# Nico59000/Ternary-image-codec

Measured on AMD Instinct MI355X. Metric: Mpix/s encode+decode 8K RS(26,20), higher is better.
Workload: dtype u8

## Files before the change

### ternary-image-codec_amd/csrc/t3_api_decode.cpp

```cpp
#include <hip/hip_runtime.h>
#include <math.h>
#include <stdio.h>
#include <string.h>

#include <stdlib.h>

#include <algorithm>
#include <mutex>
#include <vector>

#include "../../include/t3hip.h"
#include "t3_ctx.hpp"
#include "t3_decode.h"
#include "t3_host.hpp"
#include "t3_repair.h"
#include "t3_window.h"

using namespace t3;

namespace {
struct HdrCheck { HdrExpect ex; uint32_t hs; uint32_t* verdict; const uint8_t* in; };

int launch_hdr_compare(const HdrCheck* h, hipStream_t s) {
    if (!h) return T3_OK;
// ... 19 lines not shown
        HIPCHK(hipMemcpy(tab.synd_lut[ki], img.data(), tab.synd_lut_bytes[ki], hipMemcpyHostToDevice));
    }
    if (!tab.roots[ki]) {
        const Field& F = field(); const int t = (26 - k) / 2;
        size_t n = 1; for (int i = 0; i < t; ++i) n *= 27;
        std::vector<uint32_t> tbl(n);
        for (size_t idx = 0; idx < n; ++idx) {
            uint8_t sg[5] = {1, 0, 0, 0, 0}; { size_t v = idx; for (int q = 1; q <= t; ++q) { sg[q] = (uint8_t)(v % 27); v /= 27; } }
            uint32_t mask = 0;
            for (int i = 0; i < 26; ++i) {
                const uint8_t x = F.t.exp[i == 0 ? 0 : 26 - i];
                uint8_t acc = sg[t];
                for (int q = t - 1; q >= 0; --q) acc = F.t.add[F.t.mul[acc * 27 + x] * 27 + sg[q]];
                if (acc == 0) mask |= 1u << i;
            }
            tbl[idx] = mask;
        }
        HIPCHK(hipMalloc((void**)&tab.roots[ki], n * 4));
        HIPCHK(hipMemcpy(tab.roots[ki], tbl.data(), n * 4, hipMemcpyHostToDevice));
    }
    if (!tab.synd_afrag[ki]) {
        std::vector<uint32_t> af; build_mfma_syndrome(k, af);
        HIPCHK(hipMalloc((void**)&tab.synd_afrag[ki], af.size() * 4)); HIPCHK(hipMemcpy(tab.synd_afrag[ki], af.data(), af.size() * 4, hipMemcpyHostToDevice));
    }
    if (!tab.synd_T) {
        std::vector<uint32_t> img; build_syndrome_T(img);
        HIPCHK(hipMalloc((void**)&tab.synd_T, img.size() * 4)); HIPCHK(hipMemcpy(tab.synd_T, img.data(), img.size() * 4, hipMemcpyHostToDevice));
        build_syndrome_T(img, 16);
        HIPCHK(hipMalloc((void**)&tab.synd_T16, img.size() * 4)); HIPCHK(hipMemcpy(tab.synd_T16, img.data(), img.size() * 4, hipMemcpyHostToDevice));
        uint8_t sm[kFx2SmallBytes + kFx2ModBytes]; build_fx2_small(sm); build_fx2_mod(sm + kFx2SmallBytes);
        HIPCHK(hipMalloc((void**)&tab.fx2_small, sizeof sm)); HIPCHK(hipMemcpy(tab.fx2_small, sm, sizeof sm, hipMemcpyHostToDevice));
    }
    if (!tab.fma) {
        const Field& F = field();
        std::vector<uint8_t> t(19696, 0);
        for (int x = 0; x < 27; ++x) for (int y = 0; y < 27; ++y) for (int c = 0; c < 27; ++c) t[(size_t)(x * 27 + y) * 27 + c] = F.t.add[c * 27 + F.t.mul[x * 27 + y]];
        HIPCHK(hipMalloc((void**)&tab.fma, t.size())); HIPCHK(hipMemcpy(tab.fma, t.data(), t.size(), hipMemcpyHostToDevice));
    }
    return T3_OK;
}

int rgb_dequant_tables(Ctx& c, const uint8_t** out) {
    uint8_t*& d = c.rgb.dequant;
    if (!d) {
        uint8_t t[328]; memset(t, 0, sizeof t);
        auto cl = [](long v) { return v < 0 ? 0 : (v > 255 ? 255 : v); };
        for (int q = 0; q <= 242; ++q) t[q] = (uint8_t)cl(lround(q * (255.0 / 242.0)));
        for (int q = -40; q <= 40; ++q) t[244 + q + 40] = (uint8_t)cl(lround(128 + q * (128.0 / 40.0)));
        HIPCHK(hipMalloc((void**)&d, sizeof t)); HIPCHK(hipMemcpy(d, t, sizeof t, hipMemcpyHostToDevice));
    }
    *out = d; return T3_OK;
}

template <class A> void scrambler_rows(A& a, const ScrCycle& sc) {
    uint8_t rows[12][16]; memset(rows, 0, sizeof rows);
    for (int r = 0; r < 11; ++r) for (int q = 0; q < 13; ++q) rows[r][q] = (uint8_t)(27u * sc.cyc[(r + q) % 6]);
    for (int q = 0; q < 13; ++q) rows[11][q] = (uint8_t)(27u * (q == 0 ? sc.pre[0] : q == 1 ? sc.pre[1] : sc.cyc[(4 + q) % 6]));
    static_assert(sizeof a.pat == sizeof rows, "pattern rows");
    memcpy(a.pat, rows, sizeof rows);
}


struct FusedPlan { DecFx2Args a; const void* fn; uint32_t grid, threads; bool tickets, whole_frame; };
int plan_fixed_fused(uint64_t body_bytes, uint32_t hdr_syms, const t3_layout& L, const ScrCycle& sc, void* d_out, uint64_t units, int to_pixels,
                     uint32_t* d_fail, FusedPlan& p, uint32_t bcn_slot = 0, uint32_t bcn_period = 0, uint32_t tile_lo = 0, uint32_t tile_hi = 0xFFFFFFFFu) {
    if (L.interleave2d || L.n_raw_words == 0) return 1;
    Ctx& c = ctx(); const DecodeTables& tab = c.dec;
    std::lock_guard<std::mutex> lk(c.tab_mu);
    if (!single_k(L)) return 1;
// ... 820 lines not shown
```

### ternary-image-codec_amd/csrc/t3_decode_fx2.h

```cpp
#pragma once
#include "t3_decode_fx.h"
#include "t3_host.hpp"

namespace t3 {
namespace {

__device__ __forceinline__ uint32_t mod26(uint32_t u) { return min(u, u + 26u); }

struct Synd { uint32_t lo, hi; };

typedef uint32_t Geo;
struct Blk { bool valid, first; uint32_t c0, off, yb; };
constexpr uint32_t kFx2Dummy = 384;

template <int R>
__device__ __forceinline__ Geo fx2_geo(const uint32_t item, const uint32_t n_items, const uint32_t nb, const DevDiv& div_nb, const uint32_t tile0, uint32_t& off0) {
    constexpr uint32_t K = 26 - R;
    const uint32_t bi = min(div_ge2(item, div_nb), 8u), m = item - bi * nb;
    const uint32_t m3 = m - 3u * ((m * 683u) >> 11);
    const Row rw = row(bi);
    uint32_t cb = rw.boff6 + 2u * m3; cb -= cb >= 6u ? 6u : 0u;
    off0 = (uint32_t)rw.body_off + 26u * (tile0 * nb + m);
    return (bi + 9u * K * m) | cb << 16 | (item < n_items ? 1u << 19 : 0u);
}
template <int R>
__device__ __forceinline__ bool fx2_has_block(const Geo g, const uint32_t tile, const uint32_t n_tiles, const uint32_t nb) {
    constexpr uint32_t K = 26 - R;
    bool v = (g >> 19) != 0u;
    if (tile + 1u >= n_tiles) {
        const uint32_t yr = g & 0xFFFFu, m = yr / (9u * K), bi = yr - 9u * K * m;
        v = v && tile * nb + m < row(bi).blocks;
    }
    return v;
}
__device__ __forceinline__ Blk fx2_block(const Geo g, const uint32_t off, const bool valid, const uint32_t u2, const uint32_t y_off) {
// ... 75 lines not shown
    const auto sw = __builtin_amdgcn_permlane32_swap(Pown, Pown, false, false);
    Synd r; r.lo = sw[0]; r.hi = sw[1];
    if constexpr (RM != R) {
        const uint64_t V = (uint64_t)sw[0] | (uint64_t)sw[1] << (8u * H);
        constexpr uint64_t M = (1ull << (8u * HB)) - 1ull;
        r.lo = (uint32_t)(V & M); r.hi = (uint32_t)((V >> (8u * HB)) & M);
    }
    return r;
}

template <int R, uint32_t SMB = 0>
__device__ __forceinline__ uint32_t fx2_single(const Synd& sy, const uint32_t yb, const uint32_t FMA) {
    constexpr uint32_t SM = SMB + kFx2Small;
    constexpr uint32_t K = 26 - R, H = R / 2;
    uint32_t lg[R]; bool ok = true;
#pragma unroll
    for (uint32_t j = 0; j < (uint32_t)R; ++j) {
        const uint32_t s = ((j < H ? sy.lo : sy.hi) >> (8u * (j % H))) & 0xFFu;
        lg[j] = lds_u8(SM + kFx2LG + s);
        ok = ok && lg[j] != 0xFFu;
    }
    const uint32_t p = mod26(lg[1] - lg[0]);
#pragma unroll
    for (uint32_t j = 1; j + 1 < (uint32_t)R; ++j) ok = ok && mod26(lg[j + 1] - lg[j]) == p;
    if (!ok) return 0u;
    if (p < K) {
        const uint32_t m = lds_u8(SM + kFx2EX + mod26(lg[0] - p));
        const uint32_t ad = yb + 9u * p;
        *T3_LDS(uint8_t, ad) = (uint8_t)lds_u8(FMA + (2u * 27u + m) * 27u + lds_u8(ad));
    }
    return 1u;
}

template <int R, uint32_t SMB = 0, bool WIDE = true>
__device__ __forceinline__ uint32_t fx2_correct(const uint32_t* S, Fix& fx, const uint32_t* __restrict__ root_tbl, const uint32_t FMA) {
    constexpr uint32_t SM = SMB + kFx2Small;
    constexpr int T = R / 2;
    auto tab = [](uint32_t idx) -> uint32_t { return lds_u8(idx); };
    uint32_t Sx[R];
#pragma unroll
    for (int j = 0; j < R; ++j) Sx[j] = __umul24(S[j], 729u) + FMA;
    uint32_t sg[T + 1], sg27[T + 1], bs27[T + 1];
#pragma unroll
    for (int i = 0; i <= T; ++i) { sg[i] = 0; sg27[i] = 0; bs27[i] = 0; }
    sg[0] = 1; sg27[0] = 27; bs27[1] = 27u * 2u;
    uint32_t L = 0;
    bool over = false;
#pragma unroll
    for (int n = 0; n < R; ++n) {
        uint32_t d = S[n];
#pragma unroll
        for (int i = 1; i <= T; ++i) if (i <= n) d = tab(Sx[n - i] + sg27[i] + d);
        const bool upd = d != 0 && 2u * L <= (uint32_t)n;
        const uint32_t dx = __umul24(d, 729u) + FMA;
        uint32_t old27[T + 1];
#pragma unroll
        for (int i = 0; i <= T; ++i) old27[i] = sg27[i];
#pragma unroll
        for (int i = 1; i <= T; ++i) if (i <= n + 1) { sg[i] = tab(dx + bs27[i] + sg[i]); sg27[i] = 27u * sg[i]; }
        const uint32_t ninv = lds_u8(SM + kFx2NINV + d), nix = __umul24(ninv, 729u) + FMA;
        uint32_t nb27[T + 1];
        nb27[0] = 0; nb27[1] = 27u * ninv;
#pragma unroll
        for (int i = 2; i <= T; ++i) nb27[i] = (i <= n + 1) ? 27u * tab(nix + old27[i - 1]) : 0u;
        if (upd) { L = (uint32_t)n + 1u - L; over = over || L > (uint32_t)T; }
#pragma unroll
        for (int i = T; i >= 1; --i) bs27[i] = upd ? nb27[i] : bs27[i - 1];
        bs27[0] = 0;
    }
    uint32_t deg = 0;
#pragma unroll
    for (int i = 1; i <= T; ++i) if (sg[i] != 0) deg = (uint32_t)i;
    if (over || deg != L) return 1u;
    uint32_t ridx = sg[T];
#pragma unroll
    for (int q = T - 1; q >= 1; --q) ridx = ridx * 27u + sg[q];
    const uint32_t roots = root_tbl[ridx];
    const uint32_t np = (uint32_t)__popc(roots);
    if (np != deg) return 1u;
    uint32_t Om[T];
#pragma unroll
    for (int q = 0; q < T; ++q) {
        uint32_t acc = S[q];
#pragma unroll
        for (int j = 1; j <= q; ++j) acc = tab(Sx[q - j] + sg27[j] + acc);
        Om[q] = acc;
    }
    uint32_t s22 = 0;
    if constexpr (T >= 2) s22 = tab(FMA + 729u + sg27[2] + sg[2]);
    const uint32_t s22_27 = 27u * s22;
    if constexpr (WIDE) {
        uint32_t r = roots, bad = 0u;
        uint32_t pe[T], xix[T];
    #pragma unroll
        for (int e = 0; e < T; ++e) {
            const bool have = (uint32_t)e < np;
            const uint32_t p = have ? (uint32_t)__ffs((int)r) - 1u : 0u; r &= r - 1u;
            pe[e] = p;
            xix[e] = __umul24(lds_u8(SM + kFx2EX + (p == 0 ? 0u : 26u - p)), 729u) + FMA;
        }
        uint32_t num[T], den[T];
    #pragma unroll
        for (int e = 0; e < T; ++e) { num[e] = Om[T - 1]; den[e] = tab(xix[e] + s22_27 + sg[1]); }
    #pragma unroll
        for (int q = T - 2; q >= 0; --q) {
    #pragma unroll
// ... 2 lines not shown
        if constexpr (T >= 4) {
    #pragma unroll
            for (int e = 0; e < T; ++e) { const uint32_t x2 = tab(xix[e] + sg27[4]); const uint32_t x3 = tab(xix[e] + 27u * x2); den[e] = tab(xix[e] + 27u * x3 + den[e]); }
        }
    #pragma unroll
        for (int e = 0; e < T; ++e) {
            const bool have = (uint32_t)e < np;
            bad |= (have && den[e] == 0u) ? 1u : 0u;
            fx.pos[e] = pe[e]; fx.mag[e] = tab(FMA + 729u * lds_u8(SM + kFx2NEG + num[e]) + 27u * lds_u8(SM + kFx2INV + den[e]));
        }
        if (bad) return 1u;
    } else {
        uint32_t r = roots;
#pragma unroll
        for (int e = 0; e < T; ++e) {
            if ((uint32_t)e < np) {
                const uint32_t p = (uint32_t)__ffs((int)r) - 1u; r &= r - 1u;
                const uint32_t xi = lds_u8(SM + kFx2EX + (p == 0 ? 0u : 26u - p));
                const uint32_t xix = __umul24(xi, 729u) + FMA;
                uint32_t num = Om[T - 1];
#pragma unroll
                for (int q = T - 2; q >= 0; --q) num = tab(xix + 27u * num + Om[q]);
                uint32_t den = tab(xix + s22_27 + sg[1]);
                if constexpr (T >= 4) { const uint32_t x2 = tab(xix + sg27[4]); const uint32_t x3 = tab(xix + 27u * x2); den = tab(xix + 27u * x3 + den); }
                if (den == 0) return 1u;
                fx.pos[e] = p; fx.mag[e] = tab(FMA + 729u * lds_u8(SM + kFx2NEG + num) + 27u * lds_u8(SM + kFx2INV + den));
            }
        }
    }
    fx.np = np;
    return 0u;
}

template <int R, uint32_t SMB = 0, bool WIDE = true>
__device__ __forceinline__ bool fx2_fix_block(const uint32_t lo, const uint32_t hi, const uint32_t yb, const uint32_t* __restrict__ root_tbl, const uint32_t FMA) {
    constexpr uint32_t K = 26 - R, H = R / 2;
    uint32_t S[R];
#pragma unroll
    for (uint32_t j = 0; j < (uint32_t)R; ++j) S[j] = ((j < H ? lo : hi) >> (8u * (j % H))) & 0xFFu;
    Fix fx; fx.np = 0;
    if (fx2_correct<R, SMB, WIDE>(S, fx, root_tbl, FMA) != 0u) return false;
    if constexpr (WIDE) {
        uint32_t ad[R / 2], yv[R / 2];
    #pragma unroll
        for (int q = 0; q < R / 2; ++q) { ad[q] = ((uint32_t)q < fx.np && fx.pos[q] < K) ? yb + 9u * fx.pos[q] : SMB + kFx2Dummy + 4u * (uint32_t)q; yv[q] = lds_u8(ad[q]); }
    #pragma unroll
        for (int q = 0; q < R / 2; ++q) yv[q] = lds_u8(FMA + (54u + fx.mag[q]) * 27u + min(yv[q], 26u));
    #pragma unroll
        for (int q = 0; q < R / 2; ++q) *T3_LDS(uint8_t, ad[q]) = (uint8_t)yv[q];
    } else {
#pragma unroll
        for (int q = 0; q < R / 2; ++q)
            if ((uint32_t)q < fx.np && fx.pos[q] < K) { const uint32_t ad = yb + 9u * fx.pos[q]; *T3_LDS(uint8_t, ad) = (uint8_t)lds_u8(FMA + (54u + fx.mag[q]) * 27u + lds_u8(ad)); }
    }
    return true;
}

template <int R, uint32_t SMB = 0, bool WIDE = true>
__device__ __forceinline__ void fx2_own_blocks(const uint32_t* __restrict__ roots, const uint32_t fma_off, uint32_t* fail, const Synd& sA, const Synd& sB, const Blk& bA, const Blk& bB, const uint32_t tag,
                                               const uint32_t lane, const uint32_t cnt_addr, const uint32_t q_off, const uint32_t qcap) {
    const uint32_t h = lane >> 5;
    Synd own; own.lo = h ? sB.lo : sA.lo; own.hi = h ? sB.hi : sA.hi;
    const bool valid = h ? bB.valid : bA.valid;
    const uint32_t yb = h ? bB.yb : bA.yb;
    bool flagged = valid && (own.lo | own.hi) != 0u;
    if (flagged) flagged = fx2_single<R, SMB>(own, yb, fma_off) == 0u;
    const uint64_t bal = __builtin_amdgcn_ballot_w64(flagged);
    if (bal != 0ull) {
        const uint32_t cnt = (uint32_t)__popcll(bal), first = (uint32_t)__builtin_ctzll(bal);
        uint32_t base = 0;
        if (__builtin_amdgcn_mbcnt_hi(~0u, __builtin_amdgcn_mbcnt_lo(~0u, 0u)) == first) base = __hip_atomic_fetch_add((uint32_t*)__builtin_assume_aligned(lds + cnt_addr, 4), cnt, __ATOMIC_RELAXED, __HIP_MEMORY_SCOPE_WORKGROUP);
        base = __builtin_amdgcn_readlane(base, (int)first);
        if (flagged) {
            const uint32_t slot = base + __builtin_amdgcn_mbcnt_hi((uint32_t)(bal >> 32), __builtin_amdgcn_mbcnt_lo((uint32_t)bal, 0u));
            if (__builtin_expect(slot < qcap, 1)) {
                *T3_LDS(u32x2, q_off + 8u * slot) = u32x2{own.lo, own.hi};
                *T3_LDS(uint16_t, q_off + 8u * qcap + 2u * slot) = (uint16_t)tag;
            } else if (!fx2_fix_block<R, SMB, WIDE>(own.lo, own.hi, yb, roots, fma_off)) atomicAdd(fail, 1u);
        }
    }
}

template <int R, uint32_t SMB = 0, bool WIDE = true>
__device__ __forceinline__ void fx2_queue_entry(const uint32_t* __restrict__ roots, const uint32_t fma_off, uint32_t* fail, const uint32_t e, const uint32_t q_off, const uint32_t qcap, const uint32_t y_off) {
    const u32x2 sy = *T3_LDS(const u32x2, q_off + 8u * e);
    const uint32_t tag = *T3_LDS(const uint16_t, q_off + 8u * qcap + 2u * e);
    if (!fx2_fix_block<R, SMB, WIDE>(sy.x, sy.y, y_off + tag, roots, fma_off)) atomicAdd(fail, 1u);
}

}
}
```

### ternary-image-codec_amd/csrc/t3_decode_uep.hip

```cpp
#include <hip/hip_runtime.h>
#include <stdint.h>

#include "../../include/t3hip.h"
#include "t3_decode.h"
#include "t3_decode_fx.h"
#include "t3_decode_fx2.h"
#include "t3_decode_wg.h"

namespace t3 {

namespace {

constexpr uint32_t kUepCnt = 144;
struct GrpRec { uint32_t r, nb, n_items, af_off, q_rel, q_cap, div_mul, div_sh; uint8_t bands[12]; uint32_t pad_; };
static_assert(sizeof(GrpRec) == 48, "group record");

__device__ __forceinline__ IlRow row_at(const DecUepArgs& a, uint32_t v) { return il_row_of<div_ge2>(v, a.n_sym, a.il_w, a.il_A, a.div_A, a.div_w); }
struct Runs { uint32_t at[3], lo[3], len[3], n; };
__device__ __forceinline__ Runs tile_runs(const DecUepArgs& a, const uint32_t S0) {
    Runs R; R.n = 0;
#pragma unroll
    for (int i = 0; i < 3; ++i) { R.at[i] = 0; R.lo[i] = 0; R.len[i] = 0; }
    const uint32_t E = min(S0 + a.TS, a.n_sym);
    if (S0 >= E) return R;
// ... 7 lines not shown
    if (!a.il_on) { push(0u, S0, E - S0); return R; }
    const IlRow r0 = row_at(a, S0), r1 = row_at(a, E - 1u);
    const uint32_t e0 = min(r0.start + r0.len, E);
    push(0u, r0.odd ? 2u * r0.start + r0.len - e0 : S0, e0 - S0);
    if (e0 < E) {
        const uint32_t c0 = max(r1.start, e0);
        push(e0 - S0, e0, c0 - e0);
        push(c0 - S0, r1.odd ? 2u * r1.start + r1.len - E : c0, E - c0);
    }
    return R;
}

__device__ __forceinline__ void px3_from_syms(const uint32_t* s, uint16_t* o) {
    const uint32_t Y0 = s[0] + 27u * (s[1] - 9u * div9(s[1])), B0 = div9(s[1]) + 3u * s[2];
    const uint32_t R0 = s[3] + 27u * (s[4] - 3u * div3(s[4])), Y1 = div3(s[4]) + 9u * s[5];
    const uint32_t B1 = s[6] + 27u * (s[7] - 3u * div3(s[7]));
    const uint32_t R1 = div3(s[7]) + 9u * (s[8] - 9u * div9(s[8]));
    const uint32_t Y2 = div9(s[8]) + 3u * s[9] + 81u * (s[10] - 3u * div3(s[10]));
    const uint32_t B2 = div3(s[10]) + 9u * (s[11] - 9u * div9(s[11])), R2 = div9(s[11]) + 3u * s[12];
    o[0] = (uint16_t)Y0; o[1] = (uint16_t)(B0 - 40u); o[2] = (uint16_t)(R0 - 40u); o[3] = (uint16_t)Y1; o[4] = (uint16_t)(B1 - 40u); o[5] = (uint16_t)(R1 - 40u);
    o[6] = (uint16_t)Y2; o[7] = (uint16_t)(B2 - 40u); o[8] = (uint16_t)(R2 - 40u);
}

template <int R, int RM, bool WIDE>
__device__ __forceinline__ void uep_pass(const DecUepArgs& a, const Geo gA, const Geo gB, const uint32_t offA, const uint32_t offB, const bool vA, const bool vB, const bool haveB,
                                         const uint32_t u2, const uint32_t y_off, const uint32_t (&LA)[4], const uint32_t (&LB)[4], const uint32_t lane,
                                         const uint32_t af_off, const uint32_t* __restrict__ roots, const uint32_t cnt_addr, const uint32_t q_off, const uint32_t q_cap, uint32_t* const failp) {
    constexpr uint32_t TCOP = 16, TBASE = kFx2TPx, MT = kFx2ModPx;
    const uint32_t h = lane >> 5;
    const Blk bA = fx2_block(gA, offA, vA, u2, y_off), bB = fx2_block(gB, offB, vB, u2, y_off);
    const Synd sA = fx2_set<R, TCOP, TBASE, MT, 0, RM>(bA, LA, lane, af_off, a.pat_off);
    Synd sB; sB.lo = 0; sB.hi = 0;
    if (haveB) sB = fx2_set<R, TCOP, TBASE, MT, 0, RM>(bB, LB, lane, af_off, a.pat_off);
    fx2_own_blocks<R, 0, WIDE>(roots, a.fma_off, failp, sA, sB, bA, bB, (h ? gB : gA) & 0xFFFFu, lane, cnt_addr, q_off, q_cap);
}
}

template <int RA, int RB>
__global__ __launch_bounds__(512, 6) void decode_uep_px_kernel(const DecUepArgs a) {
    constexpr uint32_t NW = 4;
    constexpr bool WIDE = !(RA == 6 && RB == 4);
    const uint32_t tid = threadIdx.x, lane = tid & 63u, wave = __builtin_amdgcn_readfirstlane(tid >> 6), nthr = blockDim.x;
    const Tickets tk = tickets_setup(a);
    tk.first(tid);
    uint32_t* const failp = a.verdict ? (uint32_t*)(lds + kFx2FailWg) : a.fail;
    if (tid == 0) *(uint32_t*)(lds + kFx2FailWg) = 0u;
    if (a.verdict && blockIdx.x == 0u && wave == 2u * NW - 1u) {
        uint32_t want = 0;
#pragma unroll
        for (uint32_t q = 0; q < 24; ++q) want = lane == q ? a.hx[q] : want;
        header_check_wave(a, want, lane);
    }
    if (tid == 0) {
        stage_band_rows(a);
#pragma unroll
        for (int i = 0; i < 4; ++i) *(uint32_t*)(lds + kUepCnt + 4 * i) = 0;
        *(uint32_t*)(lds + kFx2Sync) = 0; *(uint32_t*)(lds + kFx2Abort) = 0;
#pragma unroll
        for (int g = 0; g < kUepMaxGrp; ++g) {
            GrpRec r; r.r = a.grp[g].r; r.nb = a.grp[g].nb; r.n_items = a.grp[g].n_items; r.af_off = a.grp[g].af_off; r.q_rel = a.grp[g].q_rel; r.q_cap = a.grp[g].q_cap;
            r.div_mul = a.grp[g].div_nb.mul; r.div_sh = a.grp[g].div_nb.sh; r.pad_ = 0;
#pragma unroll
            for (int q = 0; q < 12; ++q) r.bands[q] = a.grp[g].bands[q];
            *(GrpRec*)(lds + a.rec_off + 48 * g) = r;
        }
#pragma unroll
        for (int i = 0; i < 8; ++i) *(uint32_t*)(lds + a.rec_off + 96 + 4 * i) = a.pair_tab[i];
// ... 62 lines not shown
                    const uint32_t q_rel = __builtin_amdgcn_readfirstlane(*(const uint32_t*)(lds + rb + 16u)), q_cap = __builtin_amdgcn_readfirstlane(*(const uint32_t*)(lds + rb + 20u));
                    const uint32_t toff = tile * 26u * nbg, u2 = 2u * mod3_u32(tile * nbg);
                    uint32_t xa = pass ? xa1 : xa0, xb = pass ? xb1 : xb0, yy = pass ? yy1 : yy0; asm volatile("" : "+v"(xa), "+v"(xb), "+v"(yy));
                    const Geo gA = geo_of(xa, yy, 0), gB = geo_of(xb, yy, 1);
                    const uint32_t oA = (xa & 0x0FFFFFFFu) + toff, oB = (xb & 0x0FFFFFFFu) + toff;
                    const bool vA = has(gA, oA, tile), vB = has(gB, oB, tile), haveB = pip + 32u < n_items;
                    const uint32_t cnt_addr = kUepCnt + 4u * (2u * buf + pgp), q_off = a.q_off + buf * a.q_stride + q_rel;
                    if (pgp == 0u) uep_pass<RA, RA, WIDE>(a, gA, gB, oA, oB, vA, vB, haveB, u2, y_off, LA, LB, lane, af_off, a.grp[0].roots, cnt_addr, q_off, q_cap, failp);
                    else uep_pass<RB, RA, WIDE>(a, gA, gB, oA, oB, vA, vB, haveB, u2, y_off, LA, LB, lane, af_off, a.grp[1].roots, cnt_addr, q_off, q_cap, failp);
                }
            }
            if (tid == 0u) tk.publish(buf, raw, nxt);
            barrier_lds();
            cur = nxt; nxt = tk.next(buf);
        }
        barrier_lds();
    } else {
        const uint32_t cw = wave - NW, ct = cw * 64u + lane;
        uint32_t prev = 0, rdv = 0;
        auto rendezvous = [&]() { consumer_rendezvous<NW>(++rdv, failp, lane); };
        for (uint32_t k = 0;; ++k) {
            if (k >= 1u) {
                const uint32_t tile = prev, buf = (k - 1u) & 1u;
                const uint32_t y_off = a.y_off + buf * a.y_stride, S0 = tile * a.TS;
                {
                    const uint32_t rb1 = a.rec_off + 48u;
                    const uint32_t capA = __builtin_amdgcn_readfirstlane(*(const uint32_t*)(lds + a.rec_off + 20u)), capB = __builtin_amdgcn_readfirstlane(*(const uint32_t*)(lds + rb1 + 20u));
                    const uint32_t qA = a.q_off + buf * a.q_stride + __builtin_amdgcn_readfirstlane(*(const uint32_t*)(lds + a.rec_off + 16u));
                    const uint32_t qB = a.q_off + buf * a.q_stride + __builtin_amdgcn_readfirstlane(*(const uint32_t*)(lds + rb1 + 16u));
                    const uint32_t QA = min(__builtin_amdgcn_readfirstlane(*(const uint32_t*)(lds + kUepCnt + 4u * (2u * buf))), capA);
                    const uint32_t QB = a.n_grp > 1u ? min(__builtin_amdgcn_readfirstlane(*(const uint32_t*)(lds + kUepCnt + 4u * (2u * buf + 1u))), capB) : 0u;
                    const uint32_t nA = (QA + 63u) / 64u, nB = (QB + 63u) / 64u;
                    for (uint32_t sl = cw; sl < nA + nB; sl += NW) {
                        if (sl < nA) { const uint32_t e = 64u * sl + lane; if (e < QA) fx2_queue_entry<RA, 0, WIDE>(a.grp[0].roots, a.fma_off, failp, e, qA, capA, y_off); }
                        else { const uint32_t e = 64u * (sl - nA) + lane; if (e < QB) fx2_queue_entry<RB, 0, WIDE>(a.grp[1].roots, a.fma_off, failp, e, qB, capB, y_off); }
                    }
                }
                rendezvous();
                if (ct < a.n_grp) *(uint32_t*)(lds + kUepCnt + 4u * (2u * buf + ct)) = 0;
                if (a.il_on) {
                    const uint32_t E = min(S0 + a.TS, a.n_sym);
                    for (uint32_t d = ct; 4u * d < a.TS; d += 64u * NW) {
                        const uint32_t v = S0 + 4u * d;
                        if (v >= E) continue;
                        const IlRow rg = row_at(a, v);
                        if (!rg.odd) continue;
                        const uint32_t lo = max(rg.start, S0), hi = min(rg.start + rg.len, E);
                        if ((hi - lo) & 3u) {
                            if (v == lo) for (uint32_t i = lo, j = hi - 1u; i < j; ++i, --j) { const uint32_t x = lds_u8(y_off + (i - S0)); *T3_LDS(uint8_t, y_off + (i - S0)) = (uint8_t)lds_u8(y_off + (j - S0)); *T3_LDS(uint8_t, y_off + (j - S0)) = (uint8_t)x; }
                            continue;
                        }
                        const uint32_t v2 = lo + hi - 4u - v;
                        if (v2 < v) continue;
                        const uint32_t x = *T3_LDS(const uint32_t, y_off + (v - S0)), y = *T3_LDS(const uint32_t, y_off + (v2 - S0));
                        *T3_LDS(uint32_t, y_off + (v - S0)) = __builtin_bswap32(y);
                        if (v2 != v) *T3_LDS(uint32_t, y_off + (v2 - S0)) = __builtin_bswap32(x);
                    }
                    rendezvous();
                }
                const Runs R = tile_runs(a, S0);
                uint32_t j0[3], nu[3], j1[3];
#pragma unroll
                for (int i = 0; i < 3; ++i) { j0[i] = (R.lo[i] + 12u) / 13u; j1[i] = (R.lo[i] + R.len[i]) / 13u; nu[i] = j1[i] > j0[i] ? (j1[i] - j0[i] + 3u) / 4u : 0u; }
                const uint32_t n01 = nu[0] + nu[1], n_all = n01 + nu[2];
                for (uint32_t e = ct; e < n_all; e += 64u * NW) {
                    const uint32_t ri = e < nu[0] ? 0u : e < n01 ? 1u : 2u;
                    const uint32_t eb = ri == 0u ? 0u : ri == 1u ? nu[0] : n01;
                    const uint32_t rj0 = ri == 0u ? j0[0] : ri == 1u ? j0[1] : j0[2], rj1 = ri == 0u ? j1[0] : ri == 1u ? j1[1] : j1[2];
// ... 69 lines not shown
```

### ternary-image-codec_amd/csrc/t3_host.cpp

```cpp
#include "t3_host.hpp"

#include <string.h>

namespace t3 {

namespace {
struct V3 { int t[3]; };
V3 to_v(int s) { return V3{{s % 3, (s / 3) % 3, (s / 9) % 3}}; }
int to_s(const V3& v) { return v.t[0] + 3 * v.t[1] + 9 * v.t[2]; }
int mul_poly(int a, int b) {
    V3 x = to_v(a), y = to_v(b);
    int c[5] = {0, 0, 0, 0, 0};
    for (int i = 0; i < 3; ++i) for (int j = 0; j < 3; ++j) c[i + j] += x.t[i] * y.t[j];
    c[2] += c[4]; c[1] += 2 * c[4];
    c[1] += c[3]; c[0] += 2 * c[3];
    return (c[0] % 3) + 3 * (c[1] % 3) + 9 * (c[2] % 3);
}
Field make_field() {
    Field f; memset(&f, 0, sizeof f);
    for (int a = 0; a < 27; ++a) {
        V3 x = to_v(a);
        for (int b = 0; b < 27; ++b) {
            V3 y = to_v(b);
            f.t.add[a * 27 + b] = (uint8_t)to_s(V3{{(x.t[0] + y.t[0]) % 3, (x.t[1] + y.t[1]) % 3, (x.t[2] + y.t[2]) % 3}});
// ... 203 lines not shown
        const int q = 4 * s + d;
        if (q >= 13 || i >= 3 * H) continue;
        const int p = 13 * kh + q, j = hh * H + i / 3, t = i % 3;
        const uint8_t g = v.P((j + 1) * p);
        uint32_t dw = 0;
        for (int tt = 0; tt < 3; ++tt) {
            const int e = tt == 0 ? 1 : tt == 1 ? 3 : 9;
            const int c = F.t.mul[e * 27 + g];
            const int tr[3] = {c % 3, (c / 3) % 3, c / 9};
            dw |= (uint32_t)(tr[t] == 2 ? 0xFFu : (uint32_t)tr[t]) << (tt == 2 ? 24 : 8 * tt);
        }
        afrag[(size_t)(s * 64 + l) * 4 + d] = dw;
    }
}
void build_syndrome_T(std::vector<uint32_t>& img, int copies) {
    const Field& F = field();
    img.assign((size_t)3 * 27 * copies, 0u);
    auto sb = [](int t) { return (uint32_t)(t == 2 ? 0xFF : t); };
    for (int st = 0; st < 3; ++st) for (int c = 0; c < 27; ++c) {
        const int d = F.t.add[c * 27 + F.t.neg[13 * st]];
        const uint32_t dw = sb(d % 3) | sb((d / 3) % 3) << 8 | (uint32_t)d << 16 | sb(d / 9) << 24;
        for (int b = 0; b < copies; ++b) img[((size_t)st * 27 + c) * copies + b] = dw;
    }
}
void build_fx2_small(uint8_t out[kFx2SmallBytes]) {
    const Field& F = field();
    memset(out, 0, kFx2SmallBytes);
    for (int x = 0; x < 27; ++x) {
        out[kFx2LG + x] = x ? (uint8_t)F.log[x] : 0xFF;
        out[kFx2INV + x] = F.t.inv[x]; out[kFx2NEG + x] = F.t.neg[x]; out[kFx2NINV + x] = F.t.neg[F.t.inv[x]];
    }
    for (int i = 0; i < 26; ++i) out[kFx2EX + i] = F.t.exp[i];
}
void build_fx2_mod(uint8_t out[kFx2ModBytes]) {
    for (int t = 0; t < 3; ++t) for (int x = 0; x < 160; ++x) out[160 * t + x] = (uint8_t)((((x - 78) % 3 + 3) % 3) * (t == 0 ? 1 : t == 1 ? 3 : 9));
}

ScrCycle scrambler_cycle_from_next(const uint8_t next[3], uint32_t s0) {
    ScrCycle c; memset(&c, 0, sizeof c);
    for (int i = 0; i < 3; ++i) c.next[i] = next[i];
    uint32_t st = s0 % 3; uint8_t seq[8];
    for (int i = 0; i < 8; ++i) { st = next[st]; seq[i] = (uint8_t)st; }
    c.pre[0] = seq[0]; c.pre[1] = seq[1];
    for (int i = 0; i < 6; ++i) c.cyc[i] = seq[2 + i];
    uint32_t f = 0; for (int i = 0; i < 6; ++i) f |= (uint32_t)c.cyc[i] << (2 * i);
    c.cyc24 = f | f << 12;
    return c;
}
ScrCycle scrambler_cycle(uint32_t a, uint32_t b, uint32_t s0) {
    uint8_t next[3];
    for (uint32_t s = 0; s < 3; ++s) next[s] = (uint8_t)((a * s + b) % 3u);
    return scrambler_cycle_from_next(next, s0);
}

void crc12(const uint8_t* msg, int n, uint8_t out[12]) {
    uint8_t r[12]; memset(r, 0, sizeof r);
    for (int i = 0; i < n + 12; ++i) {
        const int fb = ((i < n ? msg[i] : 0) + r[11]) % 3;
        for (int j = 11; j > 0; --j) r[j] = r[j - 1];
        r[0] = (uint8_t)fb;
        r[3] = (uint8_t)((r[3] + fb) % 3); r[4] = (uint8_t)((r[4] + fb) % 3); r[7] = (uint8_t)((r[7] + fb) % 3);
    }
    memcpy(out, r, 12);
}
static const int kCrcSlots[4] = {20, 21, 22, 26};
static void header_crc_of(const uint8_t s[27], uint8_t r[12]) {
// ... 188 lines not shown
```

### ternary-image-codec_amd/csrc/t3_host.hpp

```cpp
#pragma once
#include <stdint.h>
#include <vector>

#include "../../include/t3hip.h"
#include "t3_device.h"
#include "t3_rs_core.h"

namespace t3 {

struct Field {
    RsTables t;
    int16_t  log[27];
    uint8_t  exp78[78];
    uint8_t  prim;
};
const Field& field();
inline RsView rs_view(const RsTables& t) { return RsView{t.mul, t.add, t.neg, t.inv, t.exp}; }

bool valid_k(int k);
int  k_of_band_profile(uint8_t bp);
void rs_generator(int k, uint8_t* g );
void rs_parity_matrix(int k, int mode, uint8_t* P);
bool rs_decode_host(int k, uint8_t* c26, bool fixed);

struct LutGeom {
    int k, r;
    int n_dw;
    int var_dw;
    int var_off;
    int slab_bytes;
    int total_bytes;
};
LutGeom lut_geom(int k);
void build_encode_lut(int k, int mode, std::vector<uint32_t>& image);

constexpr int kMfmaLdsBytes = kMfmaTBytes + 3 * 128;
inline int mfma_scr_pos(int k) { return k == 22 ? 22 : 20; }
void build_mfma_encode(int k, int mode, std::vector<uint32_t>& afrag, std::vector<uint32_t>& lds_img);


int  syndrome_lut_slab(int k);
void build_syndrome_lut(int k, std::vector<uint32_t>& image);

constexpr int kSyndTState = 27 * 128, kSyndTBytes = 3 * kSyndTState;
constexpr int kFx2LG = 0, kFx2EX = 32, kFx2INV = 64, kFx2NEG = 96, kFx2NINV = 128, kFx2SmallBytes = 160;
void build_mfma_syndrome(int k, std::vector<uint32_t>& afrag);
void build_syndrome_T(std::vector<uint32_t>& img, int copies = 32);
void build_fx2_small(uint8_t out[kFx2SmallBytes]);
constexpr int kFx2ModBytes = 3 * 160;
void build_fx2_mod(uint8_t out[kFx2ModBytes]);

struct ScrCycle {
    uint8_t pre[2];
    uint8_t cyc[6];
    uint32_t cyc24;
    uint8_t next[3];
};
ScrCycle scrambler_cycle(uint32_t a, uint32_t b, uint32_t s0);
ScrCycle scrambler_cycle_from_next(const uint8_t next[3], uint32_t s0);
void mfma_scrambler_table(int k, const ScrCycle& sc, uint32_t out[12]);

void crc12(const uint8_t* trits, int n, uint8_t out[12]);
void header_pack(const t3_cfg& c, uint32_t frame_seq, uint32_t band_map_hash, uint8_t s[27]);
bool header_check(const uint8_t s[27]);
void header_unpack(const uint8_t s[27], t3_cfg& out, uint32_t* frame_seq, uint32_t* band_map_hash);
int  header_encode(const t3_cfg& c, uint64_t n_raw_words, uint8_t* out );
int  header_parse(const uint8_t* words, uint64_t n_words, int mode, t3_cfg& seen, uint64_t* n_raw, uint8_t next[3]);
uint8_t beacon_symbol(uint8_t profile, uint16_t frame_seq_mod, uint8_t health);

int  plan(uint64_t n_raw_words, const t3_cfg& c, t3_layout& L);
bool want_interleave(const t3_cfg& c);
struct DecLayoutCompat {
    uint64_t body_words; uint64_t band_syms[9]; uint64_t band_blocks[9]; uint64_t use_off[9]; uint64_t use_syms;
    uint8_t band_k[9]; uint64_t out_words;
};
void plan_decode_compat(uint64_t n_in_words, const t3_cfg& seen, DecLayoutCompat& D);

struct FastDiv { uint32_t mul, sh, d; };
FastDiv fastdiv(uint32_t d);
inline DevDiv to_dev(FastDiv f) { return DevDiv{f.mul, f.sh, f.d}; }

// ... 14 lines not shown
```

Measured before the change: 126,000.

## Replace Berlekamp-Massey with closed-form 3-error locator for R=6 blocks

For RS codes with six parity symbols, the iterative Berlekamp-Massey loop in fx2_correct is replaced by a closed-form determinant solution (t3_locator3) that computes the error-locator coefficients directly from the syndromes through FMA table lookups. This aims to shorten the serial dependency chain of LDS table lookups in the block-correction path. The UEP decoder opts out through a new LOC template flag, and the FMA table construction moves into a shared host helper. The closed form adds special-case branches for degree 1 and 2, which may raise divergence or register use.

```diff
diff --git a/ternary-image-codec_amd/csrc/t3_api_decode.cpp b/ternary-image-codec_amd/csrc/t3_api_decode.cpp
--- a/ternary-image-codec_amd/csrc/t3_api_decode.cpp
+++ b/ternary-image-codec_amd/csrc/t3_api_decode.cpp
@@ -75,9 +75,7 @@
         HIPCHK(hipMalloc((void**)&tab.fx2_small, sizeof sm)); HIPCHK(hipMemcpy(tab.fx2_small, sm, sizeof sm, hipMemcpyHostToDevice));
     }
     if (!tab.fma) {
-        const Field& F = field();
-        std::vector<uint8_t> t(19696, 0);
-        for (int x = 0; x < 27; ++x) for (int y = 0; y < 27; ++y) for (int c = 0; c < 27; ++c) t[(size_t)(x * 27 + y) * 27 + c] = F.t.add[c * 27 + F.t.mul[x * 27 + y]];
+        std::vector<uint8_t> t(kFx2FmaBytes, 0); build_fx2_fma(t.data());
         HIPCHK(hipMalloc((void**)&tab.fma, t.size())); HIPCHK(hipMemcpy(tab.fma, t.data(), t.size(), hipMemcpyHostToDevice));
     }
     return T3_OK;
diff --git a/ternary-image-codec_amd/csrc/t3_decode_fx2.h b/ternary-image-codec_amd/csrc/t3_decode_fx2.h
--- a/ternary-image-codec_amd/csrc/t3_decode_fx2.h
+++ b/ternary-image-codec_amd/csrc/t3_decode_fx2.h
@@ -1,6 +1,7 @@
 #pragma once
 #include "t3_decode_fx.h"
 #include "t3_host.hpp"
+#include "t3_locator.h"
 
 namespace t3 {
 namespace {
@@ -142,7 +143,7 @@
     return 1u;
 }
 
-template <int R, uint32_t SMB = 0, bool WIDE = true>
+template <int R, uint32_t SMB = 0, bool WIDE = true, bool LOC = true>
 __device__ __forceinline__ uint32_t fx2_correct(const uint32_t* S, Fix& fx, const uint32_t* __restrict__ root_tbl, const uint32_t FMA) {
     constexpr uint32_t SM = SMB + kFx2Small;
     constexpr int T = R / 2;
@@ -150,38 +151,47 @@
     uint32_t Sx[R];
 #pragma unroll
     for (int j = 0; j < R; ++j) Sx[j] = __umul24(S[j], 729u) + FMA;
-    uint32_t sg[T + 1], sg27[T + 1], bs27[T + 1];
-#pragma unroll
-    for (int i = 0; i <= T; ++i) { sg[i] = 0; sg27[i] = 0; bs27[i] = 0; }
-    sg[0] = 1; sg27[0] = 27; bs27[1] = 27u * 2u;
-    uint32_t L = 0;
-    bool over = false;
-#pragma unroll
-    for (int n = 0; n < R; ++n) {
-        uint32_t d = S[n];
-#pragma unroll
-        for (int i = 1; i <= T; ++i) if (i <= n) d = tab(Sx[n - i] + sg27[i] + d);
-        const bool upd = d != 0 && 2u * L <= (uint32_t)n;
-        const uint32_t dx = __umul24(d, 729u) + FMA;
-        uint32_t old27[T + 1];
-#pragma unroll
-        for (int i = 0; i <= T; ++i) old27[i] = sg27[i];
-#pragma unroll
-        for (int i = 1; i <= T; ++i) if (i <= n + 1) { sg[i] = tab(dx + bs27[i] + sg[i]); sg27[i] = 27u * sg[i]; }
-        const uint32_t ninv = lds_u8(SM + kFx2NINV + d), nix = __umul24(ninv, 729u) + FMA;
-        uint32_t nb27[T + 1];
-        nb27[0] = 0; nb27[1] = 27u * ninv;
-#pragma unroll
-        for (int i = 2; i <= T; ++i) nb27[i] = (i <= n + 1) ? 27u * tab(nix + old27[i - 1]) : 0u;
-        if (upd) { L = (uint32_t)n + 1u - L; over = over || L > (uint32_t)T; }
-#pragma unroll
-        for (int i = T; i >= 1; --i) bs27[i] = upd ? nb27[i] : bs27[i - 1];
-        bs27[0] = 0;
-    }
-    uint32_t deg = 0;
-#pragma unroll
-    for (int i = 1; i <= T; ++i) if (sg[i] != 0) deg = (uint32_t)i;
-    if (over || deg != L) return 1u;
+    uint32_t sg[T + 1], sg27[T + 1];
+    uint32_t L = 0, deg = 0;
+    if constexpr (R == 6 && LOC) {
+        static_assert(kLocINV == (uint32_t)kFx2INV && kLocNEG == (uint32_t)kFx2NEG && kLocNINV == (uint32_t)kFx2NINV, "small-table offsets");
+        sg[0] = 1;
+        if (t3_locator3(tab, S, Sx, FMA, SM, L, sg) != 0u) return 1u;
+        deg = L;
+#pragma unroll
+        for (int i = 0; i <= T; ++i) sg27[i] = 27u * sg[i];
+    } else {
+        uint32_t bs27[T + 1];
+#pragma unroll
+        for (int i = 0; i <= T; ++i) { sg[i] = 0; sg27[i] = 0; bs27[i] = 0; }
+        sg[0] = 1; sg27[0] = 27; bs27[1] = 27u * 2u;
+        bool over = false;
+#pragma unroll
+        for (int n = 0; n < R; ++n) {
+            uint32_t d = S[n];
+#pragma unroll
+            for (int i = 1; i <= T; ++i) if (i <= n) d = tab(Sx[n - i] + sg27[i] + d);
+            const bool upd = d != 0 && 2u * L <= (uint32_t)n;
+            const uint32_t dx = __umul24(d, 729u) + FMA;
+            uint32_t old27[T + 1];
+#pragma unroll
+            for (int i = 0; i <= T; ++i) old27[i] = sg27[i];
+#pragma unroll
+            for (int i = 1; i <= T; ++i) if (i <= n + 1) { sg[i] = tab(dx + bs27[i] + sg[i]); sg27[i] = 27u * sg[i]; }
+            const uint32_t ninv = lds_u8(SM + kFx2NINV + d), nix = __umul24(ninv, 729u) + FMA;
+            uint32_t nb27[T + 1];
+            nb27[0] = 0; nb27[1] = 27u * ninv;
+#pragma unroll
+            for (int i = 2; i <= T; ++i) nb27[i] = (i <= n + 1) ? 27u * tab(nix + old27[i - 1]) : 0u;
+            if (upd) { L = (uint32_t)n + 1u - L; over = over || L > (uint32_t)T; }
+#pragma unroll
+            for (int i = T; i >= 1; --i) bs27[i] = upd ? nb27[i] : bs27[i - 1];
+            bs27[0] = 0;
+        }
+#pragma unroll
+        for (int i = 1; i <= T; ++i) if (sg[i] != 0) deg = (uint32_t)i;
+        if (over || deg != L) return 1u;
+    }
     uint32_t ridx = sg[T];
 #pragma unroll
     for (int q = T - 1; q >= 1; --q) ridx = ridx * 27u + sg[q];
@@ -250,14 +260,14 @@
     return 0u;
 }
 
-template <int R, uint32_t SMB = 0, bool WIDE = true>
+template <int R, uint32_t SMB = 0, bool WIDE = true, bool LOC = true>
 __device__ __forceinline__ bool fx2_fix_block(const uint32_t lo, const uint32_t hi, const uint32_t yb, const uint32_t* __restrict__ root_tbl, const uint32_t FMA) {
     constexpr uint32_t K = 26 - R, H = R / 2;
     uint32_t S[R];
 #pragma unroll
     for (uint32_t j = 0; j < (uint32_t)R; ++j) S[j] = ((j < H ? lo : hi) >> (8u * (j % H))) & 0xFFu;
     Fix fx; fx.np = 0;
-    if (fx2_correct<R, SMB, WIDE>(S, fx, root_tbl, FMA) != 0u) return false;
+    if (fx2_correct<R, SMB, WIDE, LOC>(S, fx, root_tbl, FMA) != 0u) return false;
     if constexpr (WIDE) {
         uint32_t ad[R / 2], yv[R / 2];
     #pragma unroll
@@ -274,7 +284,7 @@
     return true;
 }
 
-template <int R, uint32_t SMB = 0, bool WIDE = true>
+template <int R, uint32_t SMB = 0, bool WIDE = true, bool LOC = true>
 __device__ __forceinline__ void fx2_own_blocks(const uint32_t* __restrict__ roots, const uint32_t fma_off, uint32_t* fail, const Synd& sA, const Synd& sB, const Blk& bA, const Blk& bB, const uint32_t tag,
                                                const uint32_t lane, const uint32_t cnt_addr, const uint32_t q_off, const uint32_t qcap) {
     const uint32_t h = lane >> 5;
@@ -294,17 +304,17 @@
             if (__builtin_expect(slot < qcap, 1)) {
                 *T3_LDS(u32x2, q_off + 8u * slot) = u32x2{own.lo, own.hi};
                 *T3_LDS(uint16_t, q_off + 8u * qcap + 2u * slot) = (uint16_t)tag;
-            } else if (!fx2_fix_block<R, SMB, WIDE>(own.lo, own.hi, yb, roots, fma_off)) atomicAdd(fail, 1u);
-        }
-    }
-}
-
-template <int R, uint32_t SMB = 0, bool WIDE = true>
+            } else if (!fx2_fix_block<R, SMB, WIDE, LOC>(own.lo, own.hi, yb, roots, fma_off)) atomicAdd(fail, 1u);
+        }
+    }
+}
+
+template <int R, uint32_t SMB = 0, bool WIDE = true, bool LOC = true>
 __device__ __forceinline__ void fx2_queue_entry(const uint32_t* __restrict__ roots, const uint32_t fma_off, uint32_t* fail, const uint32_t e, const uint32_t q_off, const uint32_t qcap, const uint32_t y_off) {
     const u32x2 sy = *T3_LDS(const u32x2, q_off + 8u * e);
     const uint32_t tag = *T3_LDS(const uint16_t, q_off + 8u * qcap + 2u * e);
-    if (!fx2_fix_block<R, SMB, WIDE>(sy.x, sy.y, y_off + tag, roots, fma_off)) atomicAdd(fail, 1u);
-}
-
-}
-}
+    if (!fx2_fix_block<R, SMB, WIDE, LOC>(sy.x, sy.y, y_off + tag, roots, fma_off)) atomicAdd(fail, 1u);
+}
+
+}
+}
diff --git a/ternary-image-codec_amd/csrc/t3_decode_uep.hip b/ternary-image-codec_amd/csrc/t3_decode_uep.hip
--- a/ternary-image-codec_amd/csrc/t3_decode_uep.hip
+++ b/ternary-image-codec_amd/csrc/t3_decode_uep.hip
@@ -63,7 +63,7 @@
     const Synd sA = fx2_set<R, TCOP, TBASE, MT, 0, RM>(bA, LA, lane, af_off, a.pat_off);
     Synd sB; sB.lo = 0; sB.hi = 0;
     if (haveB) sB = fx2_set<R, TCOP, TBASE, MT, 0, RM>(bB, LB, lane, af_off, a.pat_off);
-    fx2_own_blocks<R, 0, WIDE>(roots, a.fma_off, failp, sA, sB, bA, bB, (h ? gB : gA) & 0xFFFFu, lane, cnt_addr, q_off, q_cap);
+    fx2_own_blocks<R, 0, WIDE, false>(roots, a.fma_off, failp, sA, sB, bA, bB, (h ? gB : gA) & 0xFFFFu, lane, cnt_addr, q_off, q_cap);
 }
 }
 
@@ -192,8 +192,8 @@
                     const uint32_t QB = a.n_grp > 1u ? min(__builtin_amdgcn_readfirstlane(*(const uint32_t*)(lds + kUepCnt + 4u * (2u * buf + 1u))), capB) : 0u;
                     const uint32_t nA = (QA + 63u) / 64u, nB = (QB + 63u) / 64u;
                     for (uint32_t sl = cw; sl < nA + nB; sl += NW) {
-                        if (sl < nA) { const uint32_t e = 64u * sl + lane; if (e < QA) fx2_queue_entry<RA, 0, WIDE>(a.grp[0].roots, a.fma_off, failp, e, qA, capA, y_off); }
-                        else { const uint32_t e = 64u * (sl - nA) + lane; if (e < QB) fx2_queue_entry<RB, 0, WIDE>(a.grp[1].roots, a.fma_off, failp, e, qB, capB, y_off); }
+                        if (sl < nA) { const uint32_t e = 64u * sl + lane; if (e < QA) fx2_queue_entry<RA, 0, WIDE, false>(a.grp[0].roots, a.fma_off, failp, e, qA, capA, y_off); }
+                        else { const uint32_t e = 64u * (sl - nA) + lane; if (e < QB) fx2_queue_entry<RB, 0, WIDE, false>(a.grp[1].roots, a.fma_off, failp, e, qB, capB, y_off); }
                     }
                 }
                 rendezvous();
diff --git a/ternary-image-codec_amd/csrc/t3_host.cpp b/ternary-image-codec_amd/csrc/t3_host.cpp
--- a/ternary-image-codec_amd/csrc/t3_host.cpp
+++ b/ternary-image-codec_amd/csrc/t3_host.cpp
@@ -259,6 +259,11 @@
     }
     for (int i = 0; i < 26; ++i) out[kFx2EX + i] = F.t.exp[i];
 }
+void build_fx2_fma(uint8_t out[kFx2FmaBytes]) {
+    const Field& F = field();
+    memset(out, 0, kFx2FmaBytes);
+    for (int x = 0; x < 27; ++x) for (int y = 0; y < 27; ++y) for (int c = 0; c < 27; ++c) out[(size_t)(x * 27 + y) * 27 + c] = F.t.add[c * 27 + F.t.mul[x * 27 + y]];
+}
 void build_fx2_mod(uint8_t out[kFx2ModBytes]) {
     for (int t = 0; t < 3; ++t) for (int x = 0; x < 160; ++x) out[160 * t + x] = (uint8_t)((((x - 78) % 3 + 3) % 3) * (t == 0 ? 1 : t == 1 ? 3 : 9));
 }
diff --git a/ternary-image-codec_amd/csrc/t3_host.hpp b/ternary-image-codec_amd/csrc/t3_host.hpp
--- a/ternary-image-codec_amd/csrc/t3_host.hpp
+++ b/ternary-image-codec_amd/csrc/t3_host.hpp
@@ -47,6 +47,8 @@
 void build_mfma_syndrome(int k, std::vector<uint32_t>& afrag);
 void build_syndrome_T(std::vector<uint32_t>& img, int copies = 32);
 void build_fx2_small(uint8_t out[kFx2SmallBytes]);
+constexpr int kFx2FmaBytes = 19696;
+void build_fx2_fma(uint8_t out[kFx2FmaBytes]);
 constexpr int kFx2ModBytes = 3 * 160;
 void build_fx2_mod(uint8_t out[kFx2ModBytes]);
 
diff --git a/ternary-image-codec_amd/csrc/t3_locator.h b/ternary-image-codec_amd/csrc/t3_locator.h
--- /dev/null
+++ b/ternary-image-codec_amd/csrc/t3_locator.h
@@ -0,0 +1,50 @@
+#pragma once
+#include <stdint.h>
+
+#if defined(__HIPCC__)
+#define T3_LOC_HD __host__ __device__ inline __attribute__((always_inline))
+#else
+#define T3_LOC_HD inline
+#endif
+
+namespace t3 {
+
+constexpr uint32_t kLocINV = 64, kLocNEG = 96, kLocNINV = 128;
+
+template <class Tab>
+T3_LOC_HD uint32_t t3_locator3(const Tab& tab, const uint32_t* S, const uint32_t* Sx, const uint32_t FMA, const uint32_t SM, uint32_t& L, uint32_t* sg ) {
+    const uint32_t n0 = tab(SM + kLocNEG + S[0]) * 729u + FMA, n1 = tab(SM + kLocNEG + S[1]) * 729u + FMA;
+    const uint32_t n3 = tab(SM + kLocNEG + S[3]) * 729u + FMA, n4 = tab(SM + kLocNEG + S[4]) * 729u + FMA;
+    const uint32_t A01 = tab(n0 + 27u * S[2] + tab(Sx[1] + 27u * S[1]));
+    const uint32_t A02 = tab(n0 + 27u * S[3] + tab(Sx[1] + 27u * S[2]));
+    const uint32_t A12 = tab(n1 + 27u * S[3] + tab(Sx[2] + 27u * S[2]));
+    const uint32_t a01 = 27u * A01, a02 = 27u * A02, a12 = 27u * A12;
+    const uint32_t D  = tab(Sx[4] + a01 + tab(n3 + a02 + tab(Sx[2] + a12)));
+    const uint32_t D1 = tab(Sx[5] + a01 + tab(n4 + a02 + tab(Sx[3] + a12)));
+    const uint32_t u1 = tab(tab(SM + kLocNINV + A01) * 729u + FMA + a02), u2 = tab(tab(SM + kLocINV + A01) * 729u + FMA + a12);
+    const uint32_t B01 = tab(n3 + 27u * S[3] + tab(Sx[2] + 27u * S[4]));
+    const uint32_t B02 = tab(n3 + 27u * S[4] + tab(Sx[2] + 27u * S[5]));
+    const uint32_t B12 = tab(n4 + 27u * S[4] + tab(Sx[3] + 27u * S[5]));
+    const uint32_t b01 = 27u * B01, b02 = 27u * B02, b12 = 27u * B12;
+    const uint32_t D2 = tab(Sx[2] + b01 + tab(n1 + b02 + tab(Sx[0] + b12)));
+    const uint32_t mE = tab(n3 + b01 + tab(Sx[2] + b02 + tab(n1 + b12)));
+    const uint32_t nd = tab(SM + kLocNINV + D) * 729u + FMA;
+    const uint32_t t1 = tab(nd + 27u * D1), t2 = tab(nd + 27u * D2), t3 = tab(nd + 27u * mE);
+    const bool three = D != 0u;
+    L = three ? 3u : 2u;
+    sg[1] = three ? t1 : u1; sg[2] = three ? t2 : u2; sg[3] = three ? t3 : 0u;
+    uint32_t verdict = (three ? t3 != 0u : (u2 != 0u && D1 == 0u)) ? 0u : 1u;
+    if (D == 0u && A01 == 0u) {
+        uint32_t s[6];
+        for (int j = 0; j < 6; ++j) s[j] = j < 3 ? S[j] : (Sx[j] - FMA) / 729u;
+        const uint32_t q = tab(tab(SM + kLocNINV + s[0]) * 729u + FMA + 27u * s[1]), qx = q * 729u + FMA;
+        uint32_t rest = 0u;
+        for (int n = 2; n < 6; ++n) rest |= tab(qx + 27u * s[n - 1] + s[n]);
+        const bool zero = (s[0] | s[1] | s[2] | s[3] | s[4] | s[5]) == 0u, geo = s[0] != 0u && s[1] != 0u && rest == 0u;
+        L = geo ? 1u : 0u; sg[1] = geo ? q : 0u; sg[2] = 0u; sg[3] = 0u;
+        verdict = (zero || geo) ? 0u : 1u;
+    }
+    return verdict;
+}
+
+}
```

Measured after the change: 126,700, median of 6. About the same (+0.5%).
